# mcahny/vps

Measured on NVIDIA H100. Metric: FuseTrack frame pairs/s on synthetic 1024x2048 pairs, higher is better.
Workload: dtype f32 (wgmma: 3 split-f16 products per MAC, fp32 accumulate promoted to RN register sums)

## Files before the change

### vps_b200/csrc/conv_tc32.cu

```cuda
#include "conv_tc_common.cuh"

namespace {

constexpr int T32_CONV_WARPS = 3;
constexpr int T32_KC = 32;
constexpr int T32_MAX_N = 128;
constexpr int T32_WIDE_MAX_N = 64;
constexpr int t32_threads(int nwg) { return 128 * (nwg + 1); }
constexpr int T32_STAGE_SLOTS = 2;
constexpr int T32_PLANES = 2;

__device__ unsigned int g_tc32_overflow = 0;

struct Tc32Extra {
  int rows;
  int plane_bytes;
  int stage_bytes;
  int b_plane_bytes;
  int dcn;
  int wg_n;
};

struct Tc32Share {
  int row0, c_off, n;
// ... 225 lines not shown
template <int N>
__device__ __forceinline__ void epi_tma32(const ConvTcParams& p, const Tc32Extra& e, const CUtensorMap* tmY, const float (&d)[N / 2], uint32_t box,
                                          uint32_t bias_s, float bias_v, uint32_t rbar, uint32_t rphase, int wg, int tile) {
  constexpr int BC = t32_box_c(N);
  const int i = threadIdx.x & 127, lane = threadIdx.x & 31, w = i >> 5;
  if (i < N) asm volatile("st.shared.f32 [%0], %1;" ::"r"(bias_s + 4u * i), "f"(bias_v) : "memory");
  if (i == 0) asm volatile("cp.async.bulk.wait_group.read 0;" ::: "memory");
  asm volatile("bar.sync %0, 128;" ::"r"(1 + wg) : "memory");
  if (p.res) mbar_wait(rbar, rphase);
#pragma unroll
  for (int h = 0; h < 2; ++h) {
    const int q = 16 * w + (lane >> 2) + 8 * h;
#pragma unroll
    for (int j = 0; j < N / 8; ++j) {
      const int c = 8 * j + 2 * (lane & 3);
      const uint32_t a = epi_box_addr<N>(box, q, c);
      float b0, b1, r0 = 0.f, r1 = 0.f;
      asm volatile("ld.shared.v2.f32 {%0, %1}, [%2];" : "=f"(b0), "=f"(b1) : "r"(bias_s + 4u * c));
      if (p.res) asm volatile("ld.shared.v2.f32 {%0, %1}, [%2];" : "=f"(r0), "=f"(r1) : "r"(a));
      const float2 v = epi_math(p, d[4 * j + 2 * h], d[4 * j + 2 * h + 1], b0, b1, r0, r1);
      asm volatile("st.shared.v2.f32 [%0], {%1, %2};" ::"r"(a), "f"(v.x), "f"(v.y) : "memory");
    }
  }
  asm volatile("fence.proxy.async.shared::cta;" ::: "memory");
  asm volatile("bar.sync %0, 128;" ::"r"(1 + wg) : "memory");
  const EpiBox eb = epi_box(p, e, tile, wg);
  if (i == 0 && eb.live) {
#pragma unroll
    for (int b = 0; b < N / BC; ++b) tma_store_4d(tmY, box + (uint32_t)b * (64u * BC * 4u), eb.n0 + b * BC, eb.x0, eb.y0, eb.img);
    asm volatile("cp.async.bulk.commit_group;" ::: "memory");
  }
}

template <int N, bool TMA_EPI>
__device__ __forceinline__ void consumer32(const ConvTcParams& p, const Tc32Extra& e, const Ring32& rg, int wg, const CUtensorMap* tmY,
                                           const CUtensorMap* tmR) {
  constexpr int BC = t32_box_c(N);
  const bool leader = (threadIdx.x & 127) == 0;
  constexpr bool epi_tma = TMA_EPI;
  const Tc32Share s = tc32_share(p, e, wg);
  const uint32_t b_base = rg.b_base + (uint32_t)s.c_off * 64u;
  const uint32_t box = rg.e_base + (uint32_t)wg * (64u * N * 4u), bias_s = rg.bias_base + (uint32_t)wg * (N * 4u);
  const uint32_t rbar = rg.rfull(wg);
  uint32_t rphase = 0;
  const bool halo = p.halo != 0;
  const int ntaps = p.kh * p.kw, kw = p.kw, last_cc = p.cin_chunks - 1;
  const uint32_t a_pitch = halo ? (uint32_t)p.halo_w * 64u : 512u;
  const uint64_t a_hi = desc_hi(64u, a_pitch), b_hi = desc_hi(64u, 512u);
  const uint32_t a_wg = halo ? (uint32_t)(s.row0 >> 3) * a_pitch : (uint32_t)s.row0 * 64u;
  const uint32_t plane = (uint32_t)e.plane_bytes, b_plane = (uint32_t)e.b_plane_bytes;
  float acc[N / 2], sum[N / 2];
  RingPos ap, bp;
  for (int tile = blockIdx.x; tile < p.total_tiles; tile += gridDim.x) {
    float bias_v = 0.f;
    if (epi_tma) {
      const int c = tile_coord(p, tile).n_idx * p.block_n + tc32_share(p, e, wg).c_off + (threadIdx.x & 127);
      if (p.bias && (threadIdx.x & 127) < N && c < p.cout) bias_v = __ldg(p.bias + c);
    }
#pragma unroll
    for (int i = 0; i < N / 2; ++i) sum[i] = 0.f;
    for (int cc = 0; cc <= last_cc; ++cc) {
      const bool two = cc != last_cc || p.nk_last > 1;
      uint32_t a_item = 0;
      for (Tap tap; tap.k < ntaps; tap.next(kw)) {
        if (!halo || tap.k == 0) {
          ap.wait_full(rg.pfull(ap.slot));
          a_item = rg.a_base + ap.slot * rg.a_bytes + a_wg;
        }
        bp.wait_full(rg.bfull(bp.slot));
        const uint32_t a_addr = halo ? a_item + (uint32_t)tap.r * a_pitch + (uint32_t)tap.s * 64u : a_item;
        const uint32_t b_addr = b_base + bp.slot * rg.b_bytes;
        const uint64_t A = desc_at(a_hi, a_addr), A2 = desc_at(a_hi, a_addr + plane);
        const uint64_t B = desc_at(b_hi, b_addr), B2 = desc_at(b_hi, b_addr + b_plane);
        wg::fence();
        wg::Mma<N, true>::run(acc, A2, B, 0u);
        if (two) wg::Mma<N, true>::run(acc, A2 + 2, B + 2, 1u);
        wg::Mma<N, true>::run(acc, A, B2, 1u);
        if (two) wg::Mma<N, true>::run(acc, A + 2, B2 + 2, 1u);
        wg::commit();
        wg::wait<0>();
        wg::fence_regs(acc);
#pragma unroll
        for (int i = 0; i < N / 2; ++i) acc[i] *= T32_LO_INV;
        wg::fence();
        wg::Mma<N, true>::run(acc, A, B, 1u);
        if (two) wg::Mma<N, true>::run(acc, A + 2, B + 2, 1u);
        wg::commit();
        wg::wait<0>();
        wg::fence_regs(acc);
#pragma unroll
        for (int i = 0; i < N / 2; ++i) sum[i] += acc[i];
        const bool item_done = !halo || tap.k == ntaps - 1;
        if (leader) {
          mbar_arrive(rg.bempty(bp.slot));
          if (item_done) mbar_arrive(rg.pempty(ap.slot));
          if (epi_tma && p.res && cc == 0 && tap.k == 0) {
            asm volatile("cp.async.bulk.wait_group.read 0;" ::: "memory");
            const EpiBox eb = epi_box(p, e, tile, wg);
            if (eb.live) {
              mbar_expect_tx(rbar, 64u * N * 4u);
#pragma unroll
              for (int b = 0; b < N / BC; ++b)
                tma_load_4d(box + (uint32_t)b * (64u * BC * 4u), tmR, rbar, eb.n0 + b * BC, eb.x0, eb.y0, eb.img);
            } else {
              mbar_arrive(rbar);
            }
          }
        }
        ap.next(p.a_stages, item_done);
        bp.next(p.b_stages);
      }
    }
    if (epi_tma) {
      epi_tma32<N>(p, e, tmY, sum, box, bias_s, bias_v, rbar, rphase, wg, tile);
      if (p.res) rphase ^= 1u;
    } else {
      const Tc32Share s = tc32_share(p, e, wg);
      epi_frag<N, 4>(p, sum, tile, s.row0, s.c_off);
    }
  }
  if (epi_tma && leader) asm volatile("cp.async.bulk.wait_group 0;" ::: "memory");
}

template <int NWG, bool TMA_EPI>
__device__ __forceinline__ void consumer32_n(const ConvTcParams& p, const Tc32Extra& e, const Ring32& rg, int wg,
                                             const CUtensorMap* tmY, const CUtensorMap* tmR) {
  switch (p.block_n / e.wg_n) {
    case 16: consumer32<16, TMA_EPI>(p, e, rg, wg, tmY, tmR); break;
    case 32: consumer32<32, TMA_EPI>(p, e, rg, wg, tmY, tmR); break;
    case 64: consumer32<64, TMA_EPI>(p, e, rg, wg, tmY, tmR); break;
    default:
      if constexpr (NWG == 2 && !TMA_EPI) consumer32<T32_MAX_N, false>(p, e, rg, wg, tmY, tmR);
      else __trap();
      break;
  }
}

__device__ __forceinline__ void init_bars32(const Ring32& rg, uint32_t pfull_count, uint32_t sempty_count, uint32_t consumers) {
  for (int i = threadIdx.x & 31; i < T32_NBAR; i += 32) {
    const int kind = i / MAX_STAGES;
    const uint32_t count = kind == 1 ? sempty_count : (kind == 2 ? pfull_count : ((kind == 3 || kind == 5) ? consumers : 1u));
    mbar_init(rg.bar_base + 8u * i, count);
  }
  if ((threadIdx.x & 31) < 4) mbar_init(rg.rfull(threadIdx.x & 31), 1u);
  asm volatile("fence.mbarrier_init.release.cluster;" ::: "memory");
}

template <int NWG, bool TMA_EPI>
__global__ void __launch_bounds__(t32_threads(NWG), 1)
conv_igemm_tc32_kernel(const __grid_constant__ CUtensorMap tmA, const __grid_constant__ CUtensorMap tmB,
                       const __grid_constant__ CUtensorMap tmY, const __grid_constant__ CUtensorMap tmR, const ConvTcParams p,
                       const Tc32Extra e) {
  extern __shared__ __align__(1024) uint8_t smem_raw[];
  const Ring32 rg = ring32((smem_u32(smem_raw) + 1023u) & ~1023u, p, e, NWG, TMA_EPI, false);
  const int warp = __shfl_sync(0xffffffffu, (int)threadIdx.x >> 5, 0);
  if (warp == 0) init_bars32(rg, 32 * T32_CONV_WARPS, 32 * T32_CONV_WARPS, NWG);
  if (threadIdx.x == 32) {
    asm volatile("prefetch.tensormap [%0];" ::"l"(&tmA) : "memory");
    asm volatile("prefetch.tensormap [%0];" ::"l"(&tmB) : "memory");
    if (TMA_EPI) {
      asm volatile("prefetch.tensormap [%0];" ::"l"(&tmY) : "memory");
      if (p.res) asm volatile("prefetch.tensormap [%0];" ::"l"(&tmR) : "memory");
    }
  }
  __syncthreads();
  asm volatile("griddepcontrol.wait;" ::: "memory");
  asm volatile("griddepcontrol.launch_dependents;" ::: "memory");
  if (warp == 0) producer32(p, e, rg, &tmA, &tmB);
  else if (warp < 4) converter32(p, e, rg, (int)threadIdx.x - 32, 32 * T32_CONV_WARPS);
  else consumer32_n<NWG, TMA_EPI>(p, e, rg, (warp - 4) >> 2, &tmY, &tmR);
}

__global__ void __launch_bounds__(DCN32_THREADS, 1)
dcn_igemm_tc32_kernel(const __grid_constant__ CUtensorMap tmB, const ConvTcParams p, const Tc32Extra e, const DcnParams<float> d) {
  extern __shared__ __align__(1024) uint8_t smem_raw[];
  const Ring32 rg = ring32((smem_u32(smem_raw) + 1023u) & ~1023u, p, e, 2, false, true);
  const int warp = __shfl_sync(0xffffffffu, (int)threadIdx.x >> 5, 0);
  if (warp == 0) init_bars32(rg, (uint32_t)e.rows / 8u, 1, 2);
  if (threadIdx.x == 32) asm volatile("prefetch.tensormap [%0];" ::"l"(&tmB) : "memory");
  __syncthreads();
  asm volatile("griddepcontrol.wait;" ::: "memory");
  asm volatile("griddepcontrol.launch_dependents;" ::: "memory");
  if (warp >= 4 && warp < 12) {
    asm volatile("setmaxnreg.inc.sync.aligned.u32 %0;" ::"n"(DCN32_HI_REGS));
    const int wg = (warp - 4) >> 2;
    switch (p.block_n / e.wg_n) {
      case 16: consumer32<16, false>(p, e, rg, wg, nullptr, nullptr); break;
      case 32: consumer32<32, false>(p, e, rg, wg, nullptr, nullptr); break;
      case 64: consumer32<64, false>(p, e, rg, wg, nullptr, nullptr); break;
      default: consumer32<DCN32_MAX_N, false>(p, e, rg, wg, nullptr, nullptr); break;
    }
  } else {
    asm volatile("setmaxnreg.dec.sync.aligned.u32 %0;" ::"n"(DCN32_LO_REGS));
    if (warp == 0) producer32(p, e, rg, &tmB, &tmB);
    else dcn_gather32(p, e, d, rg, rg.setup_base, rg.unit_ctr(), warp < 4 ? (int)threadIdx.x - 32 : (int)threadIdx.x - 384 + 96);
  }
}

__global__ void pack_weights_tc32_kernel(const float* __restrict__ src, const float* __restrict__ scale, unsigned short* __restrict__ bm,
                                         unsigned short* __restrict__ bl, int cout, int cin, int kh, int kw, int cout_pad,
                                         int cin_pad, int transposed) {
  const int64_t total = (int64_t)cout_pad * kh * kw * cin_pad;
  bool over = false;
// ... 6 lines not shown
    bl[i] = l;
  }
  if (over) atomicAdd(&g_tc32_overflow, 1u);
}

inline int64_t plane_elems(int cout, int cin, int kh, int kw) {
  const int64_t cout_pad = (cout + 15) / 16 * 16, cin_pad = (cin + T32_KC - 1) / T32_KC * T32_KC;
  return cout_pad * kh * kw * cin_pad;
}

bool encode_weights_tc32(CUtensorMap* m, const void* w, int nprob, int cout, int taps, int cin_pad, int block_n, const char* who) {
  const auto encode = vps::tensor_map_encoder();
  if (!encode) return false;
  const int cout_pad = (cout + 15) / 16 * 16;
  const int64_t n_plane = (int64_t)cout_pad * taps * cin_pad;
  cuuint64_t dims[5] = {(cuuint64_t)cin_pad, (cuuint64_t)cout_pad, (cuuint64_t)taps, (cuuint64_t)nprob, T32_PLANES};
  cuuint64_t strides[4] = {(cuuint64_t)taps * cin_pad * 2, (cuuint64_t)cin_pad * 2, (cuuint64_t)n_plane * 2,
                           (cuuint64_t)n_plane * nprob * 2};
  cuuint32_t box[5] = {(cuuint32_t)T32_KC, (cuuint32_t)block_n, 1, 1, T32_PLANES};
  cuuint32_t estr[5] = {1, 1, 1, 1, 1};
  const CUresult r = encode(m, CU_TENSOR_MAP_DATA_TYPE_UINT16, 5, (void*)w, dims, strides, box, estr, CU_TENSOR_MAP_INTERLEAVE_NONE,
                            CU_TENSOR_MAP_SWIZZLE_64B, CU_TENSOR_MAP_L2_PROMOTION_L2_256B, CU_TENSOR_MAP_FLOAT_OOB_FILL_NONE);
  if (r != CUDA_SUCCESS) { vps::set_error("%s: encode B failed (%d)", who, (int)r); return false; }
  return true;
}

constexpr int T32_SMEM_MAX = 227 * 1024 - 64;

struct Tc32Plan {
  ConvTcParams p;
  Tc32Extra e;
  int nwg;
  int epi_tma;
  int smem;
};

bool tc32_epi_expressible(const vps_conv_args* a, int nprob) {
  if (nprob != 1 || a->oy_mul != 1 || a->ox_mul != 1 || a->y.dtype != VPS_F32) return false;
  const int64_t px = (int64_t)a->oy_off * a->y.w + a->ox_off;
  if ((((uintptr_t)a->y.ptr + px * a->y.cs * 4) & 15) || a->y.cs % 4) return false;
  if (a->res.ptr && (a->res.dtype != VPS_F32 || (((uintptr_t)a->res.ptr + px * a->res.cs * 4) & 15) || a->res.cs % 4))
    return false;
  return true;
}

Tc32Plan tc32_tile(const vps_conv_args* a, int nprob, int nwg, int wg_n, int n) {
  Tc32Plan g = {};
  ConvTcParams& p = g.p;
  g.nwg = nwg;
  g.e.wg_n = wg_n;
  const int px = 64 * (nwg / wg_n), block_n = wg_n * n;
  p.halo = a->sh == 1 && a->sw == 1 && a->kh * a->kw > 1 && a->kh <= 8 && a->kw <= 8;
  const int tw = p.halo ? 8 : patch_tw(a->oh, a->ow, px, a->sh, a->sw);
  set_tiles(p, a, nprob, tw, px / tw, block_n, T32_KC);
  p.halo_w = tw + a->kw - 1;
  p.a_stages = p.halo ? 2 : 3;
  g.e.rows = p.halo ? (p.th + a->kh - 1) * p.halo_w : px;
  p.a_box_bytes = g.e.rows * 128;
  g.e.stage_bytes = (g.e.rows * 128 + 1023) / 1024 * 1024;
  g.e.plane_bytes = (g.e.rows * 64 + 1023) / 1024 * 1024;
  g.e.b_plane_bytes = block_n * 64;
  return g;
}

constexpr double T32_STEP_CLK = 410.0, T32_STEP_CLK_640 = 70.0, T32_MMA_CLK_N2 = 0.4, T32_CONV_CLK = 6.0, T32_B_BYTES_PER_CLK = 200.0;
int tc32_plan(const vps_conv_args* a, int nprob, Tc32Plan& out) {
  VPS_CHECK_ARG(nprob >= 1 && nprob <= MAX_PROB, "conv2d_tc32: nprob %d", nprob);
  VPS_CHECK_ARG(a->sh >= 1 && a->sh <= 2 && a->sw >= 1 && a->sw <= 2, "conv2d_tc32: stride must be 1 or 2");
  VPS_CHECK_ARG(a->kh >= 1 && a->kw >= 1 && a->cin >= 1 && a->cout >= 1 && a->oh >= 0 && a->ow >= 0 && a->x.n >= 0,
                "conv2d_tc32: bad geometry (k %dx%d, cin %d, cout %d, out %dx%d)", a->kh, a->kw, a->cin, a->cout, a->oh, a->ow);
  const int sms = vps::num_sms();
  if (sms <= 0) { vps::set_error("no device"); return VPS_E_NODEV; }
  const int cout_pad = (a->cout + 15) / 16 * 16;
  double best = -1.0;
  for (int wg_n = 1; wg_n <= 4; wg_n *= 2) {
    for (int nwg = 2; nwg <= 4; nwg += 2) {
      if (wg_n > 1 && nwg == 2) continue;
      for (int n = 16; n <= (nwg == 2 ? T32_MAX_N : T32_WIDE_MAX_N) && wg_n * n <= cout_pad; n *= 2) {
        if (cout_pad % (wg_n * n) || (wg_n > 1 && n != T32_WIDE_MAX_N)) continue;
        Tc32Plan g = tc32_tile(a, nprob, nwg, wg_n, n);
        g.p.b_stages = 2;
        if ((int)ring32(0, g.p, g.e, nwg, false, false).smem > T32_SMEM_MAX) continue;
        const int64_t tiles = g.p.total_tiles;
        const double waves = (double)((tiles + sms - 1) / sms);
        const double rows = g.p.halo ? (double)g.e.rows / (a->kh * a->kw) : (double)g.e.rows;
        const double step = T32_STEP_CLK + (nwg == 4 ? T32_STEP_CLK_640 : T32_MMA_CLK_N2 * n) + 3.0 * nwg * n + T32_CONV_CLK * rows +
                            (double)(g.p.block_n * 64 * T32_PLANES) / T32_B_BYTES_PER_CLK;
        const double t = waves * ((double)tc32_walk(g.p).steps() * step + 40.0 * n + 1500.0);
        if (best < 0 || t < best * 0.999) {
          best = t;
          out = g;
        }
      }
    }
  }
  if (best < 0) {
    vps::set_error("conv2d_tc32: ring does not fit (k %dx%d)", a->kh, a->kw);
    return VPS_E_ARG;
  }
  ConvTcParams& p = out.p;
  p.b_stages = 2;
  const auto epi_fits = [&] { return (int)ring32(0, p, out.e, out.nwg, true, false).smem <= T32_SMEM_MAX; };
  if (!p.halo && p.block_n / out.e.wg_n <= T32_EPI_MAX_N && tc32_epi_expressible(a, nprob)) {
    if (!epi_fits() && p.a_stages == 3) {
      p.a_stages = 2;
      if (!epi_fits()) p.a_stages = 3;
    }
    out.epi_tma = epi_fits();
  }
  p.b_stages = 0;
  const Ring32 rg = ring32(0, p, out.e, out.nwg, out.epi_tma, false);
  const int bst = (T32_SMEM_MAX - (int)rg.smem) / (int)rg.b_bytes;
  p.b_stages = bst > MAX_STAGES ? MAX_STAGES : bst;
  out.smem = (int)ring32(0, p, out.e, out.nwg, out.epi_tma, false).smem;
  return VPS_OK;
}

constexpr int DCN32_SMEM_MAX = 132 * 1024;
constexpr double DCN32_UNIT_CLK = 220.0, DCN32_STEP_CLK = 300.0;

// ... 84 lines not shown
                  "conv2d_tc32_multi: problems must share geometry and the packed weight buffer");
  }
  Tc32Plan g;
  int st = tc32_plan(a, nprob, g);
  if (st != VPS_OK) return st;
  ConvTcParams& p = g.p;
  const int halo_h = p.th + p.kh - 1;
  VPS_CHECK_ARG(p.b_stages >= 2, "conv2d_tc32: ring does not fit (%d x %d px halo, bn %d)", halo_h, p.halo_w, p.block_n);
  st = set_problems(p, args, nprob, "conv2d_tc32");
  if (st != VPS_OK) return st;
  if (p.total_tiles == 0) return VPS_OK;

  CUtensorMap tmA, tmB;
  if (!vps::encode_nhwc(&tmA, a->x, CU_TENSOR_MAP_DATA_TYPE_FLOAT32, T32_KC, p.halo ? p.halo_w : p.tw * a->sw,
                        p.halo ? halo_h : p.th * a->sh, a->sw, a->sh, CU_TENSOR_MAP_SWIZZLE_128B, CU_TENSOR_MAP_L2_PROMOTION_L2_128B,
                        "conv2d_tc32: encode A"))
    return VPS_E_CUDA;
  if (!encode_weights_tc32(&tmB, a->w, nprob, a->cout, a->kh * a->kw, p.cin_chunks * T32_KC, p.block_n, "conv2d_tc32"))
    return VPS_E_CUDA;
  CUtensorMap tmY = {}, tmR = {};
  if (g.epi_tma) {
    const int bc = t32_box_c(p.block_n / g.e.wg_n), box_w = p.tw < 64 ? p.tw : 64;
    const int64_t px = (int64_t)a->oy_off * a->y.w + a->ox_off;
    for (int m = 0; m < (a->res.ptr ? 2 : 1); ++m) {
      const vps_tensor& t = m ? a->res : a->y;
      vps_tensor v = t;
      v.ptr = (float*)t.ptr + px * t.cs; v.n = a->x.n; v.h = a->oh; v.w = a->ow; v.c = a->cout;
      if (!vps::encode_nhwc(m ? &tmR : &tmY, v, CU_TENSOR_MAP_DATA_TYPE_FLOAT32, bc, box_w, 64 / box_w, 1, 1,
                            bc == 32 ? CU_TENSOR_MAP_SWIZZLE_128B : CU_TENSOR_MAP_SWIZZLE_64B, CU_TENSOR_MAP_L2_PROMOTION_L2_128B,
                            m ? "conv2d_tc32: encode residual" : "conv2d_tc32: encode output", &t))
        return VPS_E_CUDA;
    }
  }
#define VPS_TC32_LAUNCH(NWG, EPI)                                                                                              \
  launch_persistent<conv_igemm_tc32_kernel<NWG, EPI>>(p.total_tiles, t32_threads(NWG), g.smem, stream, "conv2d_tc32", tmA, tmB,  \
                                                      tmY, tmR, p, g.e)
  if (g.nwg == 4) return g.epi_tma ? VPS_TC32_LAUNCH(4, true) : VPS_TC32_LAUNCH(4, false);
  return g.epi_tma ? VPS_TC32_LAUNCH(2, true) : VPS_TC32_LAUNCH(2, false);
#undef VPS_TC32_LAUNCH
}

extern "C" int vps_conv2d_tc32(const vps_conv_args* a, void* stream) { return vps_conv2d_tc32_multi(a, 1, stream); }

extern "C" int vps_conv2d_tc32_plan(const vps_conv_args* a, int nprob, int* plan) {
  Tc32Plan g;
  const int st = tc32_plan(a, nprob, g);
  if (st != VPS_OK) return st;
  plan[0] = g.nwg; plan[1] = g.p.block_n; plan[2] = g.p.tw; plan[3] = g.p.th; plan[4] = g.p.halo; plan[5] = g.epi_tma;
  plan[6] = g.e.wg_n;
  return VPS_OK;
}


extern "C" int vps_deform_conv_tc32(const vps_tensor* x, const vps_tensor* offset, const void* w, int cout, const vps_tensor* y,
                                    void* stream) {
  VPS_CHECK_ARG(x->dtype == VPS_F32 && offset->dtype == VPS_F32 && offset->c >= 18, "deform_conv_tc32: dtypes");
  VPS_CHECK_ARG(x->c % T32_KC == 0 && x->cs % 8 == 0 && ((uintptr_t)x->ptr & 31) == 0,
                "deform_conv_tc32: x must have cin %% 32 == 0 and 32-byte aligned pixel rows (256-bit sampling loads)");
  VPS_CHECK_ARG(offset->n == x->n && offset->h == x->h && offset->w == x->w && y->n == x->n && y->h == x->h && y->w == x->w &&
                    y->c == cout, "deform_conv_tc32: shapes");
  VPS_CHECK_ARG((int64_t)x->n * x->h * x->w * x->cs < (1ll << 31), "deform_conv_tc32: tensor too large for 32-bit offsets");
  VPS_CHECK_ARG(((uintptr_t)w & 127) == 0, "deform_conv_tc32: weights not aligned");
  VPS_CHECK_ARG(y->dtype == VPS_F32, "deform_conv_tc32: y must be fp32");
  vps_conv_args a = dcn_args(*x, cout);
  a.y = *y;
  Tc32Plan g;
  int st = dcn32_plan(&a, g);
  if (st != VPS_OK) return st;
  st = set_problems(g.p, &a, 1, "deform_conv_tc32");
  if (st != VPS_OK) return st;
  if (g.p.total_tiles == 0) return VPS_OK;
  const DcnParams<float> d = {(const float*)x->ptr, (const float*)offset->ptr, x->cs, offset->cs, x->h, x->w};
  CUtensorMap tmB;
  if (!encode_weights_tc32(&tmB, w, 1, cout, 9, x->c, g.p.block_n, "deform_conv_tc32")) return VPS_E_CUDA;
  static bool carveout_set = false;
  if (!carveout_set) {
    cudaFuncSetAttribute(dcn_igemm_tc32_kernel, cudaFuncAttributePreferredSharedMemoryCarveout, 58);
    (void)cudaGetLastError();
    carveout_set = true;
  }
  return launch_persistent<dcn_igemm_tc32_kernel>(g.p.total_tiles, DCN32_THREADS, g.smem, stream, "deform_conv_tc32", tmB, g.p, g.e,
                                                  d);
// ... 12 lines not shown
```

### vps_b200/csrc/conv_tc_common.cuh

```cuda
#pragma once
#include <cuda_fp16.h>

#include "common.cuh"
#include "wgmma.cuh"

namespace {

constexpr int BLOCK_M = 128;
constexpr int MAX_STAGES = 8;

constexpr int MAX_PROB = 4;

struct ConvTcParams {
  int bk;
  int nprob, tiles_per_prob;
  int ph_[MAX_PROB], pw_[MAX_PROB], oy_off_[MAX_PROB], ox_off_[MAX_PROB];
  int n_img, oh, ow;
  int th, tw, tiles_y, tiles_x;
  int n_tiles_n, block_n;
  int kh, kw, sh, sw;
  int cin_chunks;
  int a_stages, b_stages;
  int halo;
  int halo_w;
  int a_stage_bytes;
  int a_box_bytes;
  int rowg;
  int gsub;
  int nk_last;
  int total_tiles;
  void* y;
  int y_h, y_w, y_cs, y_dtype, y_vec;
  int oy_mul, ox_mul;
  const void* res;
  int res_cs, res_dtype, res_after_act, res_vec;
  const float* bias;
  int cout;
  int act;
  float slope, out_scale;
};

#ifndef VPS_MBAR_SPIN_LOG2
#define VPS_MBAR_SPIN_LOG2 26
#endif
__device__ __forceinline__ uint32_t smem_u32(const void* p) {
  return (uint32_t)__cvta_generic_to_shared(p);
}
__device__ __forceinline__ void mbar_init(uint32_t bar, uint32_t count) {
  asm volatile("mbarrier.init.shared::cta.b64 [%0], %1;" ::"r"(bar), "r"(count) : "memory");
}
__device__ __forceinline__ void mbar_expect_tx(uint32_t bar, uint32_t bytes) {
  asm volatile("mbarrier.arrive.expect_tx.shared::cta.b64 _, [%0], %1;" ::"r"(bar), "r"(bytes)
               : "memory");
}
__device__ __forceinline__ void mbar_arrive(uint32_t bar) {
  asm volatile("mbarrier.arrive.shared::cta.b64 _, [%0];" ::"r"(bar) : "memory");
}
__device__ __forceinline__ void mbar_wait(uint32_t bar, uint32_t parity) {
  asm volatile(
      "{\n"
      ".reg .pred p;\n"
      ".reg .u32 n;\n"
      "mov.u32 n, 0;\n"
      "VPS_WAIT:\n"
      "mbarrier.try_wait.parity.shared::cta.b64 p, [%0], %1;\n"
      "@p bra.uni VPS_DONE;\n"
      "add.u32 n, n, 1;\n"
      "setp.lt.u32 p, n, %2;\n"
      "@p bra.uni VPS_WAIT;\n"
      "trap;\n"
      "VPS_DONE:\n"
      "}\n" ::"r"(bar), "r"(parity), "n"(1u << VPS_MBAR_SPIN_LOG2)
      : "memory");
}
__device__ __forceinline__ void tma_load_4d(uint32_t dst, const void* tmap, uint32_t bar, int c0, int c1,
                                            int c2, int c3) {
  asm volatile(
      "cp.async.bulk.tensor.4d.shared::cluster.global.tile.mbarrier::complete_tx::bytes [%0], [%1, {%3, "
      "%4, %5, %6}], [%2];" ::"r"(dst),
      "l"(tmap), "r"(bar), "r"(c0), "r"(c1), "r"(c2), "r"(c3)
      : "memory");
}
__device__ __forceinline__ void tma_load_5d(uint32_t dst, const void* tmap, uint32_t bar, int c0, int c1, int c2, int c3,
                                            int c4) {
  asm volatile(
      "cp.async.bulk.tensor.5d.shared::cluster.global.tile.mbarrier::complete_tx::bytes [%0], [%1, {%3, "
      "%4, %5, %6, %7}], [%2];" ::"r"(dst),
      "l"(tmap), "r"(bar), "r"(c0), "r"(c1), "r"(c2), "r"(c3), "r"(c4)
      : "memory");
// ... 320 lines not shown
```

### vps_b200/ops.py

```python
import ctypes as C
import os

import torch

from . import _lib
from ._lib import (ACT_LRELU, ACT_NONE, ACT_RELU, ACT_SIGMOID, VPS_BF16, VPS_F32, VpsConvArgs, VpsError,
                   VpsTensor, check, lib)

_DT = {torch.float32: VPS_F32, torch.bfloat16: VPS_BF16}

PROFILE = None
_NOTE = {"flops": 0, "tag": ""}
SCOPE = [""]
_real_lib = lib


class _ProfLib(object):
    def __getattr__(self, name):
        f = getattr(_real_lib(), name)
        if PROFILE is None or not name.startswith("vps_") or name in ("vps_last_error", "vps_launch_count", "vps_packed_tc_bytes"):
            return f

        def w(*a):
            s, e = torch.cuda.Event(enable_timing=True), torch.cuda.Event(enable_timing=True)
# ... 190 lines not shown
    else:
        a.w = pw.simt().data_ptr()
        check(lib().vps_conv2d_simt(C.byref(a), stream()), "conv2d_simt")
    return y


def conv2d_tc_multi(x, pws, y, pads, omaps, act=ACT_NONE, slope=0.1, out_scale=1.0, oh=None, ow=None, shared32=None):
    n = len(pws)
    arr = (VpsConvArgs * n)()
    gran = pws[0].gran()
    f32 = x.dtype == torch.float32
    for i in range(n):
        a = _conv_args(x, pws[i], y, 1, 0, act, slope, None, False, out_scale, oh, ow, omaps[i], pads[i])
        a.cin_gran = gran
        a.w = shared32.data_ptr() if f32 else pws[i].tc(gran).data_ptr()
        arr[i] = a
    if PROFILE is not None:
        _NOTE["flops"] = 2 * x.shape[0] * arr[0].oh * arr[0].ow * pws[0].cout * pws[0].cin * arr[0].kh * arr[0].kw * n
        _NOTE["tag"] = "%dx%d x%d phases %d->%d @%dx%d" % (arr[0].kh, arr[0].kw, n, pws[0].cin, pws[0].cout, arr[0].oh, arr[0].ow)
    if f32:
        check(lib().vps_conv2d_tc32_multi(arr, n, stream()), "conv2d_tc32_multi")
    else:
        check(lib().vps_conv2d_tc_multi(arr, n, stream()), "conv2d_tc_multi")
    return y


def conv2d_tc32_plan(x, pws, stride=1, pad=0, oh=None, ow=None, pads=None, y=None, res=None, omaps=None):
    pws = pws if isinstance(pws, (list, tuple)) else [pws]
    n = len(pws)
    arr = (VpsConvArgs * n)()
    for i in range(n):
        arr[i] = _conv_args(x, pws[i], x if y is None else y, stride, pad, ACT_NONE, 0.1, res, False, 1.0, oh, ow,
                            omaps[i] if omaps is not None else (1, 0, 1, 0), pads[i] if pads is not None else None)
    plan = (C.c_int * 7)()
    check(_real_lib().vps_conv2d_tc32_plan(arr, n, plan), "conv2d_tc32_plan")
    return dict(nwg=plan[0], block_n=plan[1], tw=plan[2], th=plan[3], halo=plan[4], epilogue="tma" if plan[5] else "frag",
                wg_n=plan[6], layout=(plan[0] // plan[6], plan[6]))


def conv2d_tc_plan(x, pws, stride=1, pad=0, oh=None, ow=None, pads=None, y=None, res=None, omaps=None):
    pws = pws if isinstance(pws, (list, tuple)) else [pws]
    n = len(pws)
    arr = (VpsConvArgs * n)()
    for i in range(n):
        arr[i] = _conv_args(x, pws[i], x if y is None else y, stride, pad, ACT_NONE, 0.1, res, False, 1.0, oh, ow,
                            omaps[i] if omaps is not None else (1, 0, 1, 0), pads[i] if pads is not None else None)
        arr[i].cin_gran = pws[0].gran()
    plan = (C.c_int * 10)()
    check(_real_lib().vps_conv2d_tc_plan(arr, n, plan), "conv2d_tc_plan")
    keys = ("block_n", "tw", "th", "halo", "rowg", "gsub", "bk", "a_stages", "b_stages", "total_tiles")
    return dict(zip(keys, plan))


def correlation(f1, f2, out, pad, max_disp, stride1, stride2, act=ACT_NONE, slope=0.1, impl=None):
    fn = {None: "vps_correlation", "tc": "vps_correlation_tc", "simt": "vps_correlation_simt", "tc32": "vps_correlation_tc32"}[impl]
    if PROFILE is not None:
        d = 2 * (max_disp // stride2) + 1
        _NOTE["flops"] = 2 * f1.shape[0] * f1.shape[1] * f1.shape[2] * f1.shape[3] * d * d
        _NOTE["tag"] = "corr d%d s%d C%d @%dx%d" % (max_disp, stride2, f1.shape[3], f1.shape[1], f1.shape[2])
    if impl is None and F32_TC[0] and f1.dtype == torch.float32 and f2.dtype == torch.float32 and out.dtype == torch.float32:
        c = f1.shape[3]
        if (c % 64 == 0 and c <= 256 and stride1 == 1 and pad == max_disp and (max_disp, stride2) == (20, 2)
                and vt(f1).cs % 4 == 0 and vt(f2).cs % 4 == 0 and f1.data_ptr() % 16 == 0 and f2.data_ptr() % 16 == 0):
            fn = "vps_correlation_tc32"
    if fn == "vps_correlation_tc32":
        ws = torch.empty(int(lib().vps_correlation_tc32_ws_bytes(C.byref(vt(f1)))), dtype=torch.uint8, device=f1.device)
        off = (-ws.data_ptr()) % 256
        check(lib().vps_correlation_tc32(C.byref(vt(f1)), C.byref(vt(f2)), C.byref(vt(out)), pad, max_disp, stride1, stride2,
                                         act, C.c_float(slope), C.c_void_p(ws.data_ptr() + off), stream()), "correlation_tc32")
        return out
# ... 277 lines not shown
```

### vps_b200/csrc/flow_ops.cu

```cuda
#include "common.cuh"

namespace {

constexpr int CK = 16;

template <typename T, int D, int S2>
__global__ void __launch_bounds__(256) correlation_kernel(vps::TV<const T> f1, vps::TV<const T> f2,
                                                          vps::TV<T> out, int act, float slope) {
  constexpr int R = (D - 1) / 2;
  constexpr int PW = 32 + (D - 1) * S2;
  constexpr int JT = (D + 7) / 8;
  extern __shared__ float sm[];
  float* f1s = sm;
  float* f2s = sm + CK * 32;
  const int lane = threadIdx.x & 31, w = threadIdx.x >> 5;
  const int x0 = blockIdx.x * 32, y = blockIdx.y, n = blockIdx.z;
  const int H = f1.h, W = f1.w, C = f1.c;
  float acc[JT][D];
#pragma unroll
  for (int a = 0; a < JT; ++a)
#pragma unroll
    for (int b = 0; b < D; ++b) acc[a][b] = 0.f;

  for (int c0 = 0; c0 < C; c0 += CK) {
// ... 33 lines not shown
  if (x < W) {
    const float inv = 1.f / (float)C;
    T* op = out.p + out.off(n, y, x);
#pragma unroll
    for (int jt = 0; jt < JT; ++jt) {
      const int tj = w + 8 * jt;
      if (tj < D) {
#pragma unroll
        for (int ti = 0; ti < D; ++ti) {
          float v = acc[jt][ti] * inv;
          v = vps::apply_act(v, act, slope);
          vps::stf<T>(op + tj * D + ti, v);
        }
      }
    }
  }
}

template <typename T, int D, int S2>
int launch_corr(const vps_tensor* f1, const vps_tensor* f2, const vps_tensor* out, int act, float slope,
                cudaStream_t st) {
  constexpr int PW = 32 + (D - 1) * S2;
  const int smem = (CK * 32 + CK * D * PW) * 4;
  auto kern = correlation_kernel<T, D, S2>;
  if (smem > 48 * 1024) {
    if (cudaFuncSetAttribute(kern, cudaFuncAttributeMaxDynamicSharedMemorySize, smem) != cudaSuccess) {
      vps::set_error("correlation: smem attr: %s", cudaGetErrorString(cudaGetLastError()));
      return VPS_E_CUDA;
    }
  }
  dim3 grid(vps::cdiv(f1->w, 32), f1->h, f1->n);
  kern<<<grid, 256, smem, st>>>(vps::tv<const T>(*f1), vps::tv<const T>(*f2), vps::tv<T>(*out), act, slope);
  VPS_CUDA_LAST("correlation_kernel");
  return VPS_OK;
}

template <typename T, typename TF, int V>
__global__ void resample2d_kernel(vps::TV<const T> src, vps::TV<const TF> flow, vps::TV<T> out) {
  VPS_PIX_COORDS(out, V, c, x, y, n);
  const TF* fp = flow.p + flow.off(n, y, x);
  const float dx = vps::ldf<TF>(fp), dy = vps::ldf<TF>(fp + 1);
  const float xf = (float)x + dx, yf = (float)y + dy;
  const float alpha = xf - floorf(xf), beta = yf - floorf(yf);
  const int xL = max(min((int)floorf(xf), src.w - 1), 0);
  const int xR = max(min((int)floorf(xf) + 1, src.w - 1), 0);
  const int yT = max(min((int)floorf(yf), src.h - 1), 0);
  const int yB = max(min((int)floorf(yf) + 1, src.h - 1), 0);
  float a[V], b[V], cc[V], d[V];
  vps::ldv<T, V>(src.p + src.off(n, yT, xL) + c, a);
  vps::ldv<T, V>(src.p + src.off(n, yT, xR) + c, b);
  vps::ldv<T, V>(src.p + src.off(n, yB, xL) + c, cc);
  vps::ldv<T, V>(src.p + src.off(n, yB, xR) + c, d);
#pragma unroll
  for (int j = 0; j < V; ++j) {
    float v = 0.f;
    v += (1.f - alpha) * (1.f - beta) * a[j];
    v += (alpha) * (1.f - beta) * b[j];
    v += (1.f - alpha) * (beta) * cc[j];
    v += (alpha) * (beta) * d[j];
    a[j] = v;
  }
  vps::stv<T, V>(out.p + out.off(n, y, x) + c, a);
}

template <typename T, typename TO>
__global__ void channelnorm_kernel(vps::TV<const T> a, vps::TV<const T> b, int has_b, vps::TV<TO> out,
// ... 15 lines not shown
    vps::stf<TO>(out.p + out.off(n, y, x), sqrtf(s));
  }
}

}

extern "C" int vps_correlation_tc(const vps_tensor* f1, const vps_tensor* f2, const vps_tensor* out, int pad, int max_disp,
                                  int stride1, int stride2, int act, float slope, void* stream);

extern "C" int vps_correlation_simt(const vps_tensor* f1, const vps_tensor* f2, const vps_tensor* out, int pad,
                                    int max_disp, int stride1, int stride2, int act, float slope, void* stream);

extern "C" int vps_correlation(const vps_tensor* f1, const vps_tensor* f2, const vps_tensor* out, int pad,
                               int max_disp, int stride1, int stride2, int act, float slope, void* stream) {
  const bool tc = f1->dtype == VPS_BF16 && f2->dtype == VPS_BF16 && f1->c % 64 == 0 && f1->c <= 256 && f1->cs % 8 == 0 &&
                  f2->cs % 8 == 0 && ((uintptr_t)f1->ptr & 15) == 0 && ((uintptr_t)f2->ptr & 15) == 0 && stride1 == 1 &&
                  pad == max_disp && ((max_disp == 20 && stride2 == 2) || (max_disp == 4 && stride2 == 1)) &&
                  (act == VPS_ACT_NONE || act == VPS_ACT_LRELU);
  if (tc) return vps_correlation_tc(f1, f2, out, pad, max_disp, stride1, stride2, act, slope, stream);
  return vps_correlation_simt(f1, f2, out, pad, max_disp, stride1, stride2, act, slope, stream);
}

extern "C" int vps_correlation_simt(const vps_tensor* f1, const vps_tensor* f2, const vps_tensor* out, int pad,
                                    int max_disp, int stride1, int stride2, int act, float slope, void* stream) {
  VPS_CHECK_ARG(stride1 == 1 && pad == max_disp, "correlation: only stride1=1, pad==max_displacement");
  VPS_CHECK_ARG(f1->dtype == f2->dtype && f1->dtype == out->dtype, "correlation: dtype mismatch");
  VPS_CHECK_ARG(f1->h == f2->h && f1->w == f2->w && f1->c == f2->c && out->h == f1->h && out->w == f1->w,
                "correlation: shape mismatch");
  const int R = max_disp / stride2, D = 2 * R + 1;
  VPS_CHECK_ARG(out->c == D * D, "correlation: out.c %d != %d", out->c, D * D);
  cudaStream_t st = (cudaStream_t)stream;
  if (D == 21 && stride2 == 2) {
    VPS_DISPATCH_T(f1->dtype, T, return (launch_corr<T, 21, 2>(f1, f2, out, act, slope, st)));
  } else if (D == 9 && stride2 == 1) {
    VPS_DISPATCH_T(f1->dtype, T, return (launch_corr<T, 9, 1>(f1, f2, out, act, slope, st)));
  }
  vps::set_error("correlation: unsupported (max_disp %d, stride2 %d)", max_disp, stride2);
  return VPS_E_ARG;
}

extern "C" int vps_resample2d(const vps_tensor* src, const vps_tensor* flow, const vps_tensor* out, void* stream) {
  VPS_CHECK_ARG(src->dtype == out->dtype && src->c == out->c && flow->c >= 2, "resample2d: bad args");
  VPS_CHECK_ARG(flow->h == out->h && flow->w == out->w, "resample2d: flow/out size");
  if (!((int64_t)out->n * out->h * out->w * out->c)) return VPS_OK;
  const bool vec = vps::vec_ok(*src, out->c) && vps::vec_ok(*out, out->c);
  VPS_DISPATCH_T(flow->dtype, TF, VPS_DISPATCH_V(out->dtype, vec, T, V,
      (resample2d_kernel<T, TF, V><<<vps::pix_grid(out->w, out->c / V, out->h, out->n), 256, 0, (cudaStream_t)stream>>>(
          vps::tv<const T>(*src), vps::tv<const TF>(*flow), vps::tv<T>(*out)))));
  VPS_CUDA_LAST("resample2d_kernel");
  return VPS_OK;
}

extern "C" int vps_channelnorm(const vps_tensor* a, const vps_tensor* b, const vps_tensor* out, void* stream) {
  VPS_CHECK_ARG(out->c == 1 && out->h == a->h && out->w == a->w, "channelnorm: out shape");
  if (b) VPS_CHECK_ARG(b->dtype == a->dtype && b->c == a->c && b->h == a->h && b->w == a->w, "channelnorm: b");
  const int64_t total = (int64_t)a->n * a->h * a->w;
  if (!total) return VPS_OK;
  vps_tensor bb = b ? *b : *a;
  VPS_DISPATCH_T(a->dtype, T, VPS_DISPATCH_T(out->dtype, TO,
      (channelnorm_kernel<T, TO><<<vps::grid_for(total), 256, 0, (cudaStream_t)stream>>>(
          vps::tv<const T>(*a), vps::tv<const T>(bb), b != nullptr, vps::tv<TO>(*out), total))));
  VPS_CUDA_LAST("channelnorm_kernel");
  return VPS_OK;
}

namespace {
// ... 254 lines not shown
```

Baseline: 18.06.

## Software-pipeline split-f16 wgmma steps across two accumulator sets in tc32 conv

Adds a pipelined consumer path for the 2-warpgroup, N<=64 case of the f32 split-precision implicit-GEMM conv. It double-buffers accumulators so the cross-term wgmmas of the next step are issued while the current step's main product and register sum complete. This is meant to hide the two full wgmma wait<0> stalls per step. Ring-slot releases move later, and the residual TMA load is now issued after the first step instead of during it. The planner's cost model gets a lower per-step clock for this variant so it selects it, at the cost of extra accumulator registers and more complex barrier and slot release ordering.

```diff
diff --git a/vps_b200/csrc/conv_tc32.cu b/vps_b200/csrc/conv_tc32.cu
--- a/vps_b200/csrc/conv_tc32.cu
+++ b/vps_b200/csrc/conv_tc32.cu
@@ -281,7 +281,23 @@
   }
 }
 
-template <int N, bool TMA_EPI>
+template <int N>
+__device__ __forceinline__ void load_residual32(const ConvTcParams& p, const Tc32Extra& e, const CUtensorMap* tmR, uint32_t box,
+                                                uint32_t rbar, int tile, int wg) {
+  constexpr int BC = t32_box_c(N);
+  asm volatile("cp.async.bulk.wait_group.read 0;" ::: "memory");
+  const EpiBox eb = epi_box(p, e, tile, wg);
+  if (eb.live) {
+    mbar_expect_tx(rbar, 64u * N * 4u);
+#pragma unroll
+    for (int b = 0; b < N / BC; ++b)
+      tma_load_4d(box + (uint32_t)b * (64u * BC * 4u), tmR, rbar, eb.n0 + b * BC, eb.x0, eb.y0, eb.img);
+  } else {
+    mbar_arrive(rbar);
+  }
+}
+
+template <int N, bool TMA_EPI, bool PIPE = false>
 __device__ __forceinline__ void consumer32(const ConvTcParams& p, const Tc32Extra& e, const Ring32& rg, int wg, const CUtensorMap* tmY,
                                            const CUtensorMap* tmR) {
   constexpr int BC = t32_box_c(N);
@@ -308,10 +324,68 @@
     }
 #pragma unroll
     for (int i = 0; i < N / 2; ++i) sum[i] = 0.f;
-    for (int cc = 0; cc <= last_cc; ++cc) {
-      const bool two = cc != last_cc || p.nk_last > 1;
+    if constexpr (!PIPE) {
+      for (int cc = 0; cc <= last_cc; ++cc) {
+        const bool two = cc != last_cc || p.nk_last > 1;
+        uint32_t a_item = 0;
+        for (Tap tap; tap.k < ntaps; tap.next(kw)) {
+          if (!halo || tap.k == 0) {
+            ap.wait_full(rg.pfull(ap.slot));
+            a_item = rg.a_base + ap.slot * rg.a_bytes + a_wg;
+          }
+          bp.wait_full(rg.bfull(bp.slot));
+          const uint32_t a_addr = halo ? a_item + (uint32_t)tap.r * a_pitch + (uint32_t)tap.s * 64u : a_item;
+          const uint32_t b_addr = b_base + bp.slot * rg.b_bytes;
+          const uint64_t A = desc_at(a_hi, a_addr), A2 = desc_at(a_hi, a_addr + plane);
+          const uint64_t B = desc_at(b_hi, b_addr), B2 = desc_at(b_hi, b_addr + b_plane);
+          wg::fence();
+          wg::Mma<N, true>::run(acc, A2, B, 0u);
+          if (two) wg::Mma<N, true>::run(acc, A2 + 2, B + 2, 1u);
+          wg::Mma<N, true>::run(acc, A, B2, 1u);
+          if (two) wg::Mma<N, true>::run(acc, A + 2, B2 + 2, 1u);
+          wg::commit();
+          wg::wait<0>();
+          wg::fence_regs(acc);
+  #pragma unroll
+          for (int i = 0; i < N / 2; ++i) acc[i] *= T32_LO_INV;
+          wg::fence();
+          wg::Mma<N, true>::run(acc, A, B, 1u);
+          if (two) wg::Mma<N, true>::run(acc, A + 2, B + 2, 1u);
+          wg::commit();
+          wg::wait<0>();
+          wg::fence_regs(acc);
+  #pragma unroll
+          for (int i = 0; i < N / 2; ++i) sum[i] += acc[i];
+          const bool item_done = !halo || tap.k == ntaps - 1;
+          if (leader) {
+            mbar_arrive(rg.bempty(bp.slot));
+            if (item_done) mbar_arrive(rg.pempty(ap.slot));
+            if (epi_tma && p.res && cc == 0 && tap.k == 0) {
+              asm volatile("cp.async.bulk.wait_group.read 0;" ::: "memory");
+              const EpiBox eb = epi_box(p, e, tile, wg);
+              if (eb.live) {
+                mbar_expect_tx(rbar, 64u * N * 4u);
+#pragma unroll
+                for (int b = 0; b < N / BC; ++b)
+                  tma_load_4d(box + (uint32_t)b * (64u * BC * 4u), tmR, rbar, eb.n0 + b * BC, eb.x0, eb.y0, eb.img);
+              } else {
+                mbar_arrive(rbar);
+              }
+            }
+          }
+          ap.next(p.a_stages, item_done);
+          bp.next(p.b_stages);
+        }
+      }
+    } else {
+      int cc = 0;
+      Tap tap;
       uint32_t a_item = 0;
-      for (Tap tap; tap.k < ntaps; tap.next(kw)) {
+      uint64_t A = 0, B = 0;
+      bool two = false, rel_item = false, new_item = false;
+      int rel_a = 0, rel_b = 0, new_a = 0, new_b = 0;
+      float acc2[N / 2];
+      const auto issue = [&](float (&d)[N / 2]) {
         if (!halo || tap.k == 0) {
           ap.wait_full(rg.pfull(ap.slot));
           a_item = rg.a_base + ap.slot * rg.a_bytes + a_wg;
@@ -319,45 +393,68 @@
         bp.wait_full(rg.bfull(bp.slot));
         const uint32_t a_addr = halo ? a_item + (uint32_t)tap.r * a_pitch + (uint32_t)tap.s * 64u : a_item;
         const uint32_t b_addr = b_base + bp.slot * rg.b_bytes;
-        const uint64_t A = desc_at(a_hi, a_addr), A2 = desc_at(a_hi, a_addr + plane);
-        const uint64_t B = desc_at(b_hi, b_addr), B2 = desc_at(b_hi, b_addr + b_plane);
+        two = cc != last_cc || p.nk_last > 1;
+        A = desc_at(a_hi, a_addr);
+        B = desc_at(b_hi, b_addr);
+        const uint64_t A2 = desc_at(a_hi, a_addr + plane), B2 = desc_at(b_hi, b_addr + b_plane);
         wg::fence();
-        wg::Mma<N, true>::run(acc, A2, B, 0u);
-        if (two) wg::Mma<N, true>::run(acc, A2 + 2, B + 2, 1u);
-        wg::Mma<N, true>::run(acc, A, B2, 1u);
-        if (two) wg::Mma<N, true>::run(acc, A + 2, B2 + 2, 1u);
+        wg::Mma<N, true>::run(d, A2, B, 0u);
+        if (two) wg::Mma<N, true>::run(d, A2 + 2, B + 2, 1u);
+        wg::Mma<N, true>::run(d, A, B2, 1u);
+        if (two) wg::Mma<N, true>::run(d, A + 2, B2 + 2, 1u);
         wg::commit();
+        new_item = !halo || tap.k == ntaps - 1;
+        new_a = ap.slot;
+        new_b = bp.slot;
+        ap.next(p.a_stages, new_item);
+        bp.next(p.b_stages);
+        tap.next(kw);
+        if (tap.k == ntaps) { tap = Tap(); ++cc; }
+      };
+      const auto run_main = [&](float (&d)[N / 2]) {
+        wg::fence_regs(d);
+#pragma unroll
+        for (int i = 0; i < N / 2; ++i) d[i] *= T32_LO_INV;
+        wg::fence();
+        wg::Mma<N, true>::run(d, A, B, 1u);
+        if (two) wg::Mma<N, true>::run(d, A + 2, B + 2, 1u);
+        wg::commit();
+      };
+      const auto retire = [&](float (&d)[N / 2]) {
+        wg::fence_regs(d);
+#pragma unroll
+        for (int i = 0; i < N / 2; ++i) sum[i] += d[i];
+        mbar_arrive_if(rg.bempty(rel_b), leader);
+        mbar_arrive_if(rg.pempty(rel_a), leader && rel_item);
+        rel_a = new_a; rel_b = new_b; rel_item = new_item;
+      };
+      const auto residual = [&] {
+        if (epi_tma && p.res && leader) load_residual32<N>(p, e, tmR, box, rbar, tile, wg);
+      };
+      const int steps = p.cin_chunks * ntaps;
+      issue(acc);
+      wg::wait<0>();
+      run_main(acc);
+      rel_a = new_a; rel_b = new_b; rel_item = new_item;
+      for (int k = 1;; k += 2) {
+        if (k == steps) {
+          wg::wait<0>();
+          retire(acc);
+          if (k == 1) residual();
+          break;
+        }
+        issue(acc2);
+        wg::wait<1>();
+        retire(acc);
         wg::wait<0>();
-        wg::fence_regs(acc);
-#pragma unroll
-        for (int i = 0; i < N / 2; ++i) acc[i] *= T32_LO_INV;
-        wg::fence();
-        wg::Mma<N, true>::run(acc, A, B, 1u);
-        if (two) wg::Mma<N, true>::run(acc, A + 2, B + 2, 1u);
-        wg::commit();
+        if (k == 1) residual();
+        run_main(acc2);
+        if (k + 1 == steps) { wg::wait<0>(); retire(acc2); break; }
+        issue(acc);
+        wg::wait<1>();
+        retire(acc2);
         wg::wait<0>();
-        wg::fence_regs(acc);
-#pragma unroll
-        for (int i = 0; i < N / 2; ++i) sum[i] += acc[i];
-        const bool item_done = !halo || tap.k == ntaps - 1;
-        if (leader) {
-          mbar_arrive(rg.bempty(bp.slot));
-          if (item_done) mbar_arrive(rg.pempty(ap.slot));
-          if (epi_tma && p.res && cc == 0 && tap.k == 0) {
-            asm volatile("cp.async.bulk.wait_group.read 0;" ::: "memory");
-            const EpiBox eb = epi_box(p, e, tile, wg);
-            if (eb.live) {
-              mbar_expect_tx(rbar, 64u * N * 4u);
-#pragma unroll
-              for (int b = 0; b < N / BC; ++b)
-                tma_load_4d(box + (uint32_t)b * (64u * BC * 4u), tmR, rbar, eb.n0 + b * BC, eb.x0, eb.y0, eb.img);
-            } else {
-              mbar_arrive(rbar);
-            }
-          }
-        }
-        ap.next(p.a_stages, item_done);
-        bp.next(p.b_stages);
+        run_main(acc);
       }
     }
     if (epi_tma) {
@@ -371,9 +468,18 @@
   if (epi_tma && leader) asm volatile("cp.async.bulk.wait_group 0;" ::: "memory");
 }
 
-template <int NWG, bool TMA_EPI>
+template <int NWG, bool TMA_EPI, bool PIPE>
 __device__ __forceinline__ void consumer32_n(const ConvTcParams& p, const Tc32Extra& e, const Ring32& rg, int wg,
                                              const CUtensorMap* tmY, const CUtensorMap* tmR) {
+  if constexpr (PIPE) {
+    switch (p.block_n / e.wg_n) {
+      case 16: consumer32<16, TMA_EPI, true>(p, e, rg, wg, tmY, tmR); break;
+      case 32: consumer32<32, TMA_EPI, true>(p, e, rg, wg, tmY, tmR); break;
+      case 64: consumer32<64, TMA_EPI, true>(p, e, rg, wg, tmY, tmR); break;
+      default: __trap();
+    }
+    return;
+  }
   switch (p.block_n / e.wg_n) {
     case 16: consumer32<16, TMA_EPI>(p, e, rg, wg, tmY, tmR); break;
     case 32: consumer32<32, TMA_EPI>(p, e, rg, wg, tmY, tmR); break;
@@ -395,7 +501,7 @@
   asm volatile("fence.mbarrier_init.release.cluster;" ::: "memory");
 }
 
-template <int NWG, bool TMA_EPI>
+template <int NWG, bool TMA_EPI, bool PIPE>
 __global__ void __launch_bounds__(t32_threads(NWG), 1)
 conv_igemm_tc32_kernel(const __grid_constant__ CUtensorMap tmA, const __grid_constant__ CUtensorMap tmB,
                        const __grid_constant__ CUtensorMap tmY, const __grid_constant__ CUtensorMap tmR, const ConvTcParams p,
@@ -417,7 +523,7 @@
   asm volatile("griddepcontrol.launch_dependents;" ::: "memory");
   if (warp == 0) producer32(p, e, rg, &tmA, &tmB);
   else if (warp < 4) converter32(p, e, rg, (int)threadIdx.x - 32, 32 * T32_CONV_WARPS);
-  else consumer32_n<NWG, TMA_EPI>(p, e, rg, (warp - 4) >> 2, &tmY, &tmR);
+  else consumer32_n<NWG, TMA_EPI, PIPE>(p, e, rg, (warp - 4) >> 2, &tmY, &tmR);
 }
 
 __global__ void __launch_bounds__(DCN32_THREADS, 1)
@@ -490,6 +596,7 @@
   Tc32Extra e;
   int nwg;
   int epi_tma;
+  int pipe;
   int smem;
 };
 
@@ -522,6 +629,8 @@
 }
 
 constexpr double T32_STEP_CLK = 410.0, T32_STEP_CLK_640 = 70.0, T32_MMA_CLK_N2 = 0.4, T32_CONV_CLK = 6.0, T32_B_BYTES_PER_CLK = 200.0;
+constexpr int T32_PIPE_MAX_N = 64;
+constexpr double T32_STEP_CLK_PIPE = 320.0;
 int tc32_plan(const vps_conv_args* a, int nprob, Tc32Plan& out) {
   VPS_CHECK_ARG(nprob >= 1 && nprob <= MAX_PROB, "conv2d_tc32: nprob %d", nprob);
   VPS_CHECK_ARG(a->sh >= 1 && a->sh <= 2 && a->sw >= 1 && a->sw <= 2, "conv2d_tc32: stride must be 1 or 2");
@@ -542,8 +651,9 @@
         const int64_t tiles = g.p.total_tiles;
         const double waves = (double)((tiles + sms - 1) / sms);
         const double rows = g.p.halo ? (double)g.e.rows / (a->kh * a->kw) : (double)g.e.rows;
-        const double step = T32_STEP_CLK + (nwg == 4 ? T32_STEP_CLK_640 : T32_MMA_CLK_N2 * n) + 3.0 * nwg * n + T32_CONV_CLK * rows +
-                            (double)(g.p.block_n * 64 * T32_PLANES) / T32_B_BYTES_PER_CLK;
+        g.pipe = nwg == 2 && n <= T32_PIPE_MAX_N;
+        const double step = (g.pipe ? T32_STEP_CLK_PIPE : T32_STEP_CLK) + (nwg == 4 ? T32_STEP_CLK_640 : T32_MMA_CLK_N2 * n) +
+                            3.0 * nwg * n + T32_CONV_CLK * rows + (double)(g.p.block_n * 64 * T32_PLANES) / T32_B_BYTES_PER_CLK;
         const double t = waves * ((double)tc32_walk(g.p).steps() * step + 40.0 * n + 1500.0);
         if (best < 0 || t < best * 0.999) {
           best = t;
@@ -694,11 +804,12 @@
         return VPS_E_CUDA;
     }
   }
-#define VPS_TC32_LAUNCH(NWG, EPI)                                                                                              \
-  launch_persistent<conv_igemm_tc32_kernel<NWG, EPI>>(p.total_tiles, t32_threads(NWG), g.smem, stream, "conv2d_tc32", tmA, tmB,  \
-                                                      tmY, tmR, p, g.e)
-  if (g.nwg == 4) return g.epi_tma ? VPS_TC32_LAUNCH(4, true) : VPS_TC32_LAUNCH(4, false);
-  return g.epi_tma ? VPS_TC32_LAUNCH(2, true) : VPS_TC32_LAUNCH(2, false);
+#define VPS_TC32_LAUNCH(NWG, EPI, PIPE)                                                                                        \
+  launch_persistent<conv_igemm_tc32_kernel<NWG, EPI, PIPE>>(p.total_tiles, t32_threads(NWG), g.smem, stream, "conv2d_tc32", tmA,  \
+                                                            tmB, tmY, tmR, p, g.e)
+  if (g.pipe) return g.epi_tma ? VPS_TC32_LAUNCH(2, true, true) : VPS_TC32_LAUNCH(2, false, true);
+  if (g.nwg == 4) return g.epi_tma ? VPS_TC32_LAUNCH(4, true, false) : VPS_TC32_LAUNCH(4, false, false);
+  return g.epi_tma ? VPS_TC32_LAUNCH(2, true, false) : VPS_TC32_LAUNCH(2, false, false);
 #undef VPS_TC32_LAUNCH
 }
 
@@ -709,7 +820,7 @@
   const int st = tc32_plan(a, nprob, g);
   if (st != VPS_OK) return st;
   plan[0] = g.nwg; plan[1] = g.p.block_n; plan[2] = g.p.tw; plan[3] = g.p.th; plan[4] = g.p.halo; plan[5] = g.epi_tma;
-  plan[6] = g.e.wg_n;
+  plan[6] = g.e.wg_n; plan[7] = g.pipe;
   return VPS_OK;
 }
 
diff --git a/vps_b200/csrc/conv_tc_common.cuh b/vps_b200/csrc/conv_tc_common.cuh
--- a/vps_b200/csrc/conv_tc_common.cuh
+++ b/vps_b200/csrc/conv_tc_common.cuh
@@ -55,6 +55,10 @@
 }
 __device__ __forceinline__ void mbar_arrive(uint32_t bar) {
   asm volatile("mbarrier.arrive.shared::cta.b64 _, [%0];" ::"r"(bar) : "memory");
+}
+__device__ __forceinline__ void mbar_arrive_if(uint32_t bar, bool pred) {
+  asm volatile("{\n.reg .pred p;\nsetp.ne.u32 p, %1, 0;\n@p mbarrier.arrive.shared::cta.b64 _, [%0];\n}\n" ::"r"(bar), "r"((uint32_t)pred)
+               : "memory");
 }
 __device__ __forceinline__ void mbar_wait(uint32_t bar, uint32_t parity) {
   asm volatile(
diff --git a/vps_b200/ops.py b/vps_b200/ops.py
--- a/vps_b200/ops.py
+++ b/vps_b200/ops.py
@@ -246,10 +246,10 @@
     for i in range(n):
         arr[i] = _conv_args(x, pws[i], x if y is None else y, stride, pad, ACT_NONE, 0.1, res, False, 1.0, oh, ow,
                             omaps[i] if omaps is not None else (1, 0, 1, 0), pads[i] if pads is not None else None)
-    plan = (C.c_int * 7)()
+    plan = (C.c_int * 8)()
     check(_real_lib().vps_conv2d_tc32_plan(arr, n, plan), "conv2d_tc32_plan")
     return dict(nwg=plan[0], block_n=plan[1], tw=plan[2], th=plan[3], halo=plan[4], epilogue="tma" if plan[5] else "frag",
-                wg_n=plan[6], layout=(plan[0] // plan[6], plan[6]))
+                wg_n=plan[6], layout=(plan[0] // plan[6], plan[6]), pipelined=plan[7])
 
 
 def conv2d_tc_plan(x, pws, stride=1, pad=0, oh=None, ow=None, pads=None, y=None, res=None, omaps=None):
```

Result: no change. 18.08 (median of 6 runs) (+0.1%).

## Add double-buffered float4 SIMT correlation kernel for 9x9 f32 displacement

Applied to the files above, without the earlier changes.

Adds a dedicated f32 correlation kernel for the 9x9, stride-1 case. It uses one warp per displacement row (288 threads), precomputed 128-bit global load offsets, and a register-prefetched, double-buffered shared-memory channel pipeline with padded stride. The aim is to cut the per-chunk load and sync stalls and the scalar gather overhead of the generic SIMT kernel. It takes more shared memory and registers, and it applies only to aligned inputs whose channel count is a multiple of 4. It may not run at all if the tensor-core correlation path is selected first.

```diff
diff --git a/vps_b200/csrc/flow_ops.cu b/vps_b200/csrc/flow_ops.cu
--- a/vps_b200/csrc/flow_ops.cu
+++ b/vps_b200/csrc/flow_ops.cu
@@ -89,6 +89,109 @@
   dim3 grid(vps::cdiv(f1->w, 32), f1->h, f1->n);
   kern<<<grid, 256, smem, st>>>(vps::tv<const T>(*f1), vps::tv<const T>(*f2), vps::tv<T>(*out), act, slope);
   VPS_CUDA_LAST("correlation_kernel");
+  return VPS_OK;
+}
+
+constexpr int C9_D = 9, C9_PW = 32 + C9_D - 1;
+constexpr int C9_CS = C9_D * C9_PW + 2;
+constexpr int C9_THREADS = 32 * C9_D;
+constexpr int C9_F1V = 32 * CK / 4, C9_F2V = C9_D * C9_PW * CK / 4;
+constexpr int C9_LOADS = (C9_F1V + C9_F2V + C9_THREADS - 1) / C9_THREADS;
+constexpr int C9_BUF = CK * 32 + CK * C9_CS;
+static_assert(C9_F1V % 4 == 0 && C9_THREADS % 4 == 0 && C9_THREADS >= C9_F1V,
+              "a thread's items share their 4-channel group, and only its first item can be an f1 item");
+
+__global__ void __launch_bounds__(C9_THREADS, 3) correlation9_f32_kernel(vps::TV<const float> f1, vps::TV<const float> f2,
+                                                                    vps::TV<float> out, int act, float slope) {
+  extern __shared__ float sm[];
+  const int lane = threadIdx.x & 31, w = threadIdx.x >> 5;
+  const int x0 = blockIdx.x * 32, y = blockIdx.y, n = blockIdx.z;
+  const int H = f1.h, W = f1.w, C = f1.c;
+  const int cq = 4 * (threadIdx.x & 3);
+  int off[C9_LOADS], dst[C9_LOADS];
+#pragma unroll
+  for (int k = 0; k < C9_LOADS; ++k) {
+    const int i = threadIdx.x + k * C9_THREADS;
+    off[k] = -1; dst[k] = -1;
+    if (i < C9_F1V) {
+      const int px = i >> 2, x = x0 + px;
+      dst[k] = cq * 32 + px;
+      if (x < W) off[k] = (int)f1.off(n, y, x) + cq;
+    } else if (i < C9_F1V + C9_F2V) {
+      const int t = (i - C9_F1V) >> 2, px = t % C9_PW, r = t / C9_PW;
+      const int x = x0 + px - (C9_D - 1) / 2, yy = y + r - (C9_D - 1) / 2;
+      dst[k] = CK * 32 + cq * C9_CS + r * C9_PW + px;
+      if (x >= 0 && x < W && yy >= 0 && yy < H) off[k] = (int)f2.off(n, yy, x) + cq;
+    }
+  }
+  float4 v[C9_LOADS];
+  const auto load = [&](int c0) {
+#pragma unroll
+    for (int k = 0; k < C9_LOADS; ++k) {
+      v[k] = make_float4(0.f, 0.f, 0.f, 0.f);
+      const float* base = k == 0 && threadIdx.x < C9_F1V ? f1.p : f2.p;
+      if (off[k] >= 0 && c0 + cq < C) v[k] = __ldg(reinterpret_cast<const float4*>(base + off[k] + c0));
+    }
+  };
+  const auto store = [&](float* buf) {
+#pragma unroll
+    for (int k = 0; k < C9_LOADS; ++k) {
+      if (dst[k] < 0) continue;
+      const int cs = dst[k] >= CK * 32 ? C9_CS : 32;
+      float* d = buf + dst[k];
+      d[0] = v[k].x; d[cs] = v[k].y; d[2 * cs] = v[k].z; d[3 * cs] = v[k].w;
+    }
+  };
+  float acc[C9_D];
+#pragma unroll
+  for (int t = 0; t < C9_D; ++t) acc[t] = 0.f;
+  load(0);
+  store(sm);
+  __syncthreads();
+  int b = 0;
+  for (int c0 = 0; c0 < C; c0 += CK) {
+    const bool more = c0 + CK < C;
+    if (more) load(c0 + CK);
+    const float* f1s = sm + b * C9_BUF;
+    const float* f2s = f1s + CK * 32 + w * C9_PW + lane;
+#pragma unroll 4
+    for (int c = 0; c < CK; ++c) {
+      const float a = f1s[c * 32 + lane];
+      const float* rowp = f2s + c * C9_CS;
+#pragma unroll
+      for (int ti = 0; ti < C9_D; ++ti) acc[ti] = fmaf(a, rowp[ti], acc[ti]);
+    }
+    if (more) store(sm + (b ^ 1) * C9_BUF);
+    __syncthreads();
+    b ^= 1;
+  }
+  const int x = x0 + lane;
+  if (x < W) {
+    const float inv = 1.f / (float)C;
+    float* op = out.p + out.off(n, y, x);
+#pragma unroll
+    for (int ti = 0; ti < C9_D; ++ti) {
+      float r = acc[ti] * inv;
+      r = vps::apply_act(r, act, slope);
+      vps::stf<float>(op + w * C9_D + ti, r);
+    }
+  }
+}
+
+int launch_corr9_f32(const vps_tensor* f1, const vps_tensor* f2, const vps_tensor* out, int act, float slope, cudaStream_t st) {
+  constexpr int smem = 2 * C9_BUF * 4;
+  static bool smem_raised = false;
+  if (!smem_raised) {
+    if (cudaFuncSetAttribute(correlation9_f32_kernel, cudaFuncAttributeMaxDynamicSharedMemorySize, smem) != cudaSuccess) {
+      vps::set_error("correlation: smem attr: %s", cudaGetErrorString(cudaGetLastError()));
+      return VPS_E_CUDA;
+    }
+    smem_raised = true;
+  }
+  dim3 grid(vps::cdiv(f1->w, 32), f1->h, f1->n);
+  correlation9_f32_kernel<<<grid, C9_THREADS, smem, st>>>(vps::tv<const float>(*f1), vps::tv<const float>(*f2), vps::tv<float>(*out),
+                                                          act, slope);
+  VPS_CUDA_LAST("correlation9_f32_kernel");
   return VPS_OK;
 }
 
@@ -170,6 +273,10 @@
   cudaStream_t st = (cudaStream_t)stream;
   if (D == 21 && stride2 == 2) {
     VPS_DISPATCH_T(f1->dtype, T, return (launch_corr<T, 21, 2>(f1, f2, out, act, slope, st)));
+  } else if (D == C9_D && stride2 == 1 && f1->dtype == VPS_F32 && f1->c % 4 == 0 && f1->cs % 4 == 0 && f2->cs % 4 == 0 &&
+             ((uintptr_t)f1->ptr & 15) == 0 && ((uintptr_t)f2->ptr & 15) == 0 &&
+             (int64_t)f1->n * f1->h * f1->w * f1->cs < (1ll << 31) && (int64_t)f2->n * f2->h * f2->w * f2->cs < (1ll << 31)) {
+    return launch_corr9_f32(f1, f2, out, act, slope, st);
   } else if (D == 9 && stride2 == 1) {
     VPS_DISPATCH_T(f1->dtype, T, return (launch_corr<T, 9, 1>(f1, f2, out, act, slope, st)));
   }
```

Result: faster. 17.86 before, 18.17 after (median of 6 runs) (+1.7%).
